# jihun1998/AO

Measured on AMD Instinct MI355X. Metric: points/sec fwd+bwd PTv2m2 S3DIS, higher is better.
Workload: dtype fp32

## Files before the change

ao_amd/csrc/abi.hip:

```cpp
#include <algorithm>
#include <cstdlib>
#include <cstring>
#include <mutex>
#include <unordered_map>
#include <vector>

#include "gva_common.h"

extern "C" int ptv2_abi_version(void) { return 11; }

extern "C" long long ptv2_struct_bytes(int which) {
    switch (which) {
        case 0: return (long long)sizeof(ptv2_block);
        case 1: return (long long)sizeof(ptv2_block_grads);
        case 2: return (long long)sizeof(ptv2_model);
        case 3: return (long long)sizeof(ptv2_gva_block);
        case 4: return (long long)sizeof(ptv2_scene_geo);
        default: return -1;
    }
}

namespace { thread_local int g_matmul_bf16 = 0; }
int ptv2_matmul_bf16(void) { return g_matmul_bf16; }
void ptv2_set_matmul_bf16(int on) { g_matmul_bf16 = on ? 1 : 0; }
// ... 74 lines not shown
        if (ids[r] < 0 || ids[r] >= dst_rows) return PTV2_ERR_ARG;
    for (long long r = 0; r < rows; ++r) memcpy(dst + ids[r] * c, src + r * c, sizeof(float) * (size_t)c);
    return PTV2_OK;
}

namespace {
std::mutex g_cnt_mu;
struct CounterKey {
    int device;
    hipStream_t stream;
    bool operator==(const CounterKey &o) const { return device == o.device && stream == o.stream; }
};
struct CounterKeyHash {
    size_t operator()(const CounterKey &k) const { return std::hash<void *>()((void *)k.stream) * 31u + (size_t)k.device; }
};
std::unordered_map<CounterKey, unsigned *, CounterKeyHash> g_counters;
}

unsigned *ptv2_stream_counters(hipStream_t st) {
    int device = 0;
    if (hipGetDevice(&device) != hipSuccess) return nullptr;
    std::lock_guard<std::mutex> lk(g_cnt_mu);
    const CounterKey key{device, st};
    auto it = g_counters.find(key);
    if (it != g_counters.end()) return it->second;
    unsigned *p = nullptr;
    if (hipMalloc((void **)&p, sizeof(unsigned) * PTV2_NUM_COUNTERS) != hipSuccess) return nullptr;
    if (hipMemsetAsync(p, 0, sizeof(unsigned) * PTV2_NUM_COUNTERS, st) != hipSuccess) return nullptr;
    g_counters[key] = p;
    return p;
}

namespace {
const char *kNames[KID_COUNT] = {
    "knn_row_query_kernel [family]", "logits_fwd_kernel [family]", "softmax_rows_kernel [family]", "aggregate_tile_kernel [family]",
    "peb_fwd_kernel [family]", "peb_bwd_kernel<8>", "aggregate_bwd_tile_kernel [family]", "aggregate_bwd_rows_kernel [family]",
    "aggregate_bwd_gv_kernel<8>", "logits_bwd_rows_kernel [family]", "logits_bwd_gather_kernel", "logits_bwd_params_kernel [family]",
    "linear_wgrad_kernel [family]", "bn_stats_kernel", "bn_apply_kernel [family]", "bn_bwd_reduce_kernel [family]",
    "bn_bwd_apply_kernel [family]", "skinny_fwd_kernel", "skinny_bwd_kernel", "rows_gemm_kernel<48, false, 32> [family]",
    "rows_gemm_kernel<48, false, 64> [family]", "rows_gemm_kernel<48, true, 32> [family]", "rows_gemm_kernel<48, true, 64> [family]",
    "rows_gemm_kernel<64, false, 32> [family]", "rows_gemm_kernel<64, false, 64> [family]", "rows_gemm_kernel<64, true, 32> [family]",
    "rows_gemm_kernel<64, true, 64> [family]",
    "attention_bwd_point_kernel<6, 48, 1, true>",
    "attention_bwd_point_kernel<12, 96, 1, false>", "attention_bwd_point_kernel<24, 192, 2, false>",
    "attention_bwd_point_kernel<48, 384, 4, false>", "attention_bwd_point_kernel<64, 512, 4, false>",
    "linear_wgrad_lds_kernel [family]",
    "grouped_wgrad_kernel_jobs", "attention_fwd_point6_kernel",
    "logits_bwd_fused6_kernel<48>", "logits_bwd_fused_kernel<12, 96, 1>", "logits_bwd_fused_kernel<24, 192, 4>",
    "logits_bwd_fused_kernel<48, 384, 4>", "logits_bwd_fused_kernel<64, 512, 4>",
    "bn_bwd_apply_residual_kernel", "bn_bwd_finapply_kernel [family]",
    "attention_fwd_tile_kernel<12, 96, 12>", "attention_fwd_tile_kernel<24, 192, 12>", "attention_fwd_tile_kernel<48, 384, 12>",
    "attention_fwd_tile_kernel<64, 512, 16>", "wp2_wgrad_tile_kernel_jobs",
    "attention_bwd_tile_kernel<12, 96, 8>", "attention_bwd_tile_kernel<24, 192, 8>", "attention_bwd_tile_kernel<48, 384, 8>",
    "attention_bwd_tile_kernel<64, 512, 8>"};
struct Rec { hipEvent_t a, b; double bytes; };
std::mutex g_mu;
int g_on = 0;
int g_only = -1;
int g_stride = 1;
unsigned g_seen[KID_COUNT];
std::vector<hipEvent_t> g_free;
hipEvent_t take_event() {
    if (!g_free.empty()) { hipEvent_t e = g_free.back(); g_free.pop_back(); return e; }
    hipEvent_t e = nullptr;
    if (hipEventCreate(&e) != hipSuccess) return nullptr;
    return e;
}
std::vector<Rec> g_recs[KID_COUNT];
std::vector<hipEvent_t> g_pending[KID_COUNT];
constexpr int STAMP_CAP = 1 << 15;
unsigned long long *g_stamp_buf = nullptr;
double g_stamp_us_per_tick = 0.01;
int g_stamp_n = 0;
struct StampRec { int slot; double bytes; };
std::vector<StampRec> g_stamp_recs[KID_COUNT];
std::vector<int> g_stamp_pending[KID_COUNT];
unsigned g_scope_period[GRAPH_SLOTS][KID_COUNT];
unsigned g_scope_phase[GRAPH_SLOTS];
thread_local unsigned t_scope_seen[KID_COUNT];
thread_local int t_scope_which = -1;
__global__ void stamp_kernel(unsigned long long *p) {
    if (threadIdx.x == 0) *p = wall_clock64();
}
}

extern "C" int ptv2_profile_is_on(void) { return g_on; }
int ptv2_profile_stamps(void) { return g_on && g_only >= 0 && g_stamp_buf != nullptr; }
void ptv2_profile_scope(int which, int end, int ring_entry, int ring_size) {
    if (which < 0 || which >= GRAPH_SLOTS) return;
    std::lock_guard<std::mutex> lk(g_mu);
    if (!end) {
        for (int k = 0; k < KID_COUNT; ++k) t_scope_seen[k] = 0;
        t_scope_which = which;
        const int stride = g_stride > 1 ? g_stride : 1;
        g_scope_phase[which] = (unsigned)(ring_entry * std::max(1, stride / std::max(1, ring_size)));
    } else {
        for (int k = 0; k < KID_COUNT; ++k) g_scope_period[which][k] = t_scope_seen[k];
        t_scope_which = -1;
    }
}
int ptv2_profile_wants(int kid) {
    if (!g_on || (g_only >= 0 && g_only != kid)) return 0;
    std::lock_guard<std::mutex> lk(g_mu);
    if (ptv2_graph_capturing() && t_scope_which >= 0) {
        const unsigned o = t_scope_seen[kid]++, P = g_scope_period[t_scope_which][kid], ph = g_scope_phase[t_scope_which];
        const unsigned stride = g_stride > 1 ? (unsigned)g_stride : 1u;
        return (P > 0 ? ((o + ph) % P) % stride : o % stride) == 0;
// ... 136 lines not shown
```

ao_amd/csrc/common.h:

```cpp
#pragma once
#include <hip/hip_runtime.h>
#include <stdint.h>
#include <stdlib.h>

#include "../../include/ptv2_hip.h"

#define WAVE 64

#define PTV2_CHECK_LAUNCH()                         \
    do {                                            \
        if (hipGetLastError() != hipSuccess) return PTV2_ERR_LAUNCH; \
    } while (0)

#define RUN(call)                        \
    do {                                 \
        int rc_ = (call);                \
        if (rc_ != PTV2_OK) return rc_;  \
    } while (0)

static inline int divup(long long a, long long b) { return (int)((a + b - 1) / b); }

static constexpr size_t ptv2_align256(size_t v) { return (v + 255) & ~(size_t)255; }
struct PtvCarver {
    char *p; size_t off;
    char *take(size_t bytes) { char *r = p ? p + off : nullptr; off += ptv2_align256(bytes); return r; }
    template <class T> T *take_n(size_t count) { return (T *)take(sizeof(T) * count); }
};

static inline bool ptv2_env_set(const char *name) { return getenv(name) != nullptr; }
static inline bool ptv2_env_is(const char *name, char c) { const char *e = getenv(name); return e && e[0] == c; }

enum PtvKernelId {
    KID_KNN_QUERY = 0, KID_LOGITS_FWD, KID_SOFTMAX_ROWS, KID_AGG_TILE, KID_PEB_FWD, KID_PEB_BWD, KID_BWD_TILE,
    KID_BWD_ROWS, KID_BWD_GV, KID_LOGITS_BWD_ROWS, KID_LOGITS_BWD_GATHER, KID_LOGITS_BWD_PARAMS, KID_WGRAD,
    KID_BN_STATS, KID_BN_APPLY, KID_BN_BWD_REDUCE, KID_BN_BWD_APPLY, KID_SKINNY_FWD, KID_SKINNY_BWD, KID_ROWS_GEMM,  KID_BWD_POINT = KID_ROWS_GEMM + 8,
     KID_WGRAD_LDS = KID_BWD_POINT + 5 ,
    KID_WGRAD_GROUPED ,
    KID_FWD_POINT ,
    KID_LOGITS_BWD_FUSED ,
    KID_BN_BWD_APPLY_RES = KID_LOGITS_BWD_FUSED + 5 ,
    KID_BN_BWD_FINAPPLY ,
    KID_FWD_TILE ,
    KID_WGRAD_TILE = KID_FWD_TILE + 4 ,
    KID_BWD_TILE_K ,
    KID_COUNT = KID_BWD_TILE_K + 4
};
extern "C" int ptv2_profile_is_on(void);
int ptv2_profile_wants(int kid);
void ptv2_profile_begin(int kid, hipStream_t st);
void ptv2_profile_end(int kid, hipStream_t st, double algorithmic_bytes);
struct PtvScopedTimer {
    int kid; hipStream_t st; double bytes; bool on;
    PtvScopedTimer(int k, hipStream_t s, double b) : kid(k), st(s), bytes(b), on(ptv2_profile_wants(k) != 0) {
        if (on) ptv2_profile_begin(kid, st);
    }
    ~PtvScopedTimer() { if (on) ptv2_profile_end(kid, st, bytes); }
};

enum PtvGraphSlot { GRAPH_MODEL_FWD = 0, GRAPH_MODEL_BWD = 1, GRAPH_MODEL_FWD_PREFIX = 2, GRAPH_MODEL_FWD_REST = 3, GRAPH_SLOTS = 4 };
struct PtvGraphScope {
    void *st, *cap; int which, ring_entry; bool active; long long t0;
    PtvGraphScope(void *stream, int which, bool allow = true);
    void *stream() const { return cap; }
    int finish(int rc);
    ~PtvGraphScope();
    PtvGraphScope(const PtvGraphScope &) = delete;
    PtvGraphScope &operator=(const PtvGraphScope &) = delete;
};
int ptv2_graph_capturing(void);
int ptv2_profile_stamps(void);
int ptv2_zero_async(void *p, size_t bytes, hipStream_t st);

void ptv2_wgrad_defer_begin(void *arena, size_t bytes);
bool ptv2_wgrad_defer_active();
float *ptv2_wgrad_defer_alloc(size_t floats);
void ptv2_wgrad_defer_arm(bool on);
void ptv2_wgrad_defer_arm_rs(bool on);
bool ptv2_wgrad_defer_armed_rs();
int ptv2_wgrad_defer_flush(void *stream);
void ptv2_wgrad_defer_end();
size_t ptv2_wgrad_defer_table_bytes();

int ptv2_matmul_bf16(void);
void ptv2_set_matmul_bf16(int on);
struct PtvMatmulScope {
    int prev;
    explicit PtvMatmulScope(int on) : prev(ptv2_matmul_bf16()) { ptv2_set_matmul_bf16(on); }
    ~PtvMatmulScope() { ptv2_set_matmul_bf16(prev); }
};
typedef __bf16 ptv2_bf16x8 __attribute__((ext_vector_type(8)));
__device__ __forceinline__ ptv2_bf16x8 ptv2_pack_bf16(float4 lo, float4 hi) {
    ptv2_bf16x8 r;
    r[0] = (__bf16)lo.x; r[1] = (__bf16)lo.y; r[2] = (__bf16)lo.z; r[3] = (__bf16)lo.w;
    r[4] = (__bf16)hi.x; r[5] = (__bf16)hi.y; r[6] = (__bf16)hi.z; r[7] = (__bf16)hi.w;
    return r;
}

static __device__ __attribute__((aligned(16), unused)) float ptv2_zero_pad[1024];
// ... 45 lines not shown
```

ao_amd/csrc/gemm.hip:

```cpp
#include <algorithm>

#include "common.h"

namespace gemm {

constexpr int BM = 64;
constexpr int THREADS = 256;
template <int KC>
__device__ __forceinline__ int lds_slot(int row, int k4) {
    return row * (KC + 8) + 4 * (k4 ^ (row & (KC == 32 ? 1 : 3)));
}

typedef float v4f __attribute__((ext_vector_type(4)));

struct GemmMulti {
    const float *X[3], *W[3], *bias[3];
    float *Y[3];
    int count;
    int sum;
    const float *xsc, *xsh;
    float *stats[3];
    const float *bnx, *bnm, *bnr, *bng, *bnb;
    int bnrelu;
    float *brec;
};

template <int CTRL>
__device__ __forceinline__ float dpp_mov(float v) {
    return __int_as_float(__builtin_amdgcn_update_dpp(0, __float_as_int(v), CTRL, 0xF, 0xF, true));
}
__device__ __forceinline__ float row16_sum(float v) {
    v += dpp_mov<0xB1>(v);
    v += dpp_mov<0x4E>(v);
    v += dpp_mov<0x141>(v);
    v += dpp_mov<0x140>(v);
    return v;
}

template <int BN>
__device__ __forceinline__ void gemm_epilogue(v4f (&acc)[BN / 16], const long long row0, const int rb, const int n0, const int z,
                                              const bool indep, const int m, const int n, const float *__restrict__ bias,
                                              float *__restrict__ Y, const int accumulate, const GemmMulti &multi, float *sS_) {
    constexpr int NT = BN / 16;
    const int tid = threadIdx.x, lane = tid & 63, wid = tid >> 6;
    float *sX = sS_;
    const long long row = row0 + wid * 16 + (lane & 15);
    float4 val[NT];
#pragma unroll
    for (int t = 0; t < NT; ++t) {
        const int col = n0 + t * 16 + (lane >> 4) * 4;
        float4 v = make_float4(acc[t][0], acc[t][1], acc[t][2], acc[t][3]);
        {
            const float4 bb = ptv2_ld_or_zero((const float4 *)(bias + col), bias && col < n);
            v.x += bb.x; v.y += bb.y; v.z += bb.z; v.w += bb.w;
        }
        val[t] = v;
        if (row < m && col < n) {
            float4 *dst = (float4 *)(Y + row * n + col);
            if (accumulate) {
                const float4 o = *dst;
                v.x += o.x; v.y += o.y; v.z += o.z; v.w += o.w;
            }
            *dst = v;
        }
    }
    if (multi.count && multi.brec) {
        float *sS = sX;
        const bool rv = row < m;
        const int cl = (lane >> 4) * 4;
        __syncthreads();
#pragma unroll
        for (int t = 0; t < NT; ++t) {
            const int col = n0 + t * 16 + cl;
            float4 d = make_float4(0.f, 0.f, 0.f, 0.f), e = d;
            if (rv && col < n) {
                const float4 xv = *(const float4 *)(multi.bnx + row * n + col);
                const float4 mm = *(const float4 *)(multi.bnm + col), rs = *(const float4 *)(multi.bnr + col);
                float4 h;
                h.x = (xv.x - mm.x) * rs.x; h.y = (xv.y - mm.y) * rs.y; h.z = (xv.z - mm.z) * rs.z; h.w = (xv.w - mm.w) * rs.w;
                d = val[t];
                if (multi.bnrelu) {
                    const float4 gg = *(const float4 *)(multi.bng + col), bb = *(const float4 *)(multi.bnb + col);
                    if (__builtin_fmaf(h.x, gg.x, bb.x) <= 0.f) d.x = 0.f;
                    if (__builtin_fmaf(h.y, gg.y, bb.y) <= 0.f) d.y = 0.f;
                    if (__builtin_fmaf(h.z, gg.z, bb.z) <= 0.f) d.z = 0.f;
                    if (__builtin_fmaf(h.w, gg.w, bb.w) <= 0.f) d.w = 0.f;
                }
                e = make_float4(d.x * h.x, d.y * h.y, d.z * h.z, d.w * h.w);
            }
            const float ax = row16_sum(d.x), ay = row16_sum(d.y), az = row16_sum(d.z), aw = row16_sum(d.w);
            const float bx = row16_sum(e.x), by = row16_sum(e.y), bz = row16_sum(e.z), bw = row16_sum(e.w);
            if ((lane & 15) == 0) {
                *(float4 *)(sS + (wid * 2 + 0) * BN + t * 16 + cl) = make_float4(ax, ay, az, aw);
                *(float4 *)(sS + (wid * 2 + 1) * BN + t * 16 + cl) = make_float4(bx, by, bz, bw);
            }
        }
        __syncthreads();
        for (int e = tid; e < 2 * BN; e += THREADS) {
            const int which = e / BN, cc = e - which * BN;
            if (n0 + cc < n) {
                float a = sS[which * BN + cc];
#pragma unroll
                for (int w = 1; w < 4; ++w) a += sS[(w * 2 + which) * BN + cc];
                multi.brec[(size_t)rb * 2 * n + (size_t)which * n + n0 + cc] = a;
            }
        }
// ... 1 lines not shown
    float *stats = multi.count ? multi.stats[indep ? z : 0] : nullptr;
    if (stats) {
        float *sS = sX;
        const bool rv = row < m;
        const int cnt = (int)((m - row0) < BM ? (m - row0) : BM);
        const int cl = (lane >> 4) * 4;
        __syncthreads();
#pragma unroll
        for (int t = 0; t < NT; ++t) {
            const float sx = row16_sum(rv ? val[t].x : 0.f), sy = row16_sum(rv ? val[t].y : 0.f);
            const float sz = row16_sum(rv ? val[t].z : 0.f), sw = row16_sum(rv ? val[t].w : 0.f);
            if ((lane & 15) == 0) *(float4 *)(sS + wid * BN + t * 16 + cl) = make_float4(sx, sy, sz, sw);
        }
        __syncthreads();
        float4 mean[NT];
#pragma unroll
        for (int t = 0; t < NT; ++t) {
            float4 a = *(const float4 *)(sS + t * 16 + cl);
#pragma unroll
            for (int w = 1; w < 4; ++w) {
                const float4 o = *(const float4 *)(sS + w * BN + t * 16 + cl);
                a.x += o.x; a.y += o.y; a.z += o.z; a.w += o.w;
            }
            mean[t] = a;
        }
        __syncthreads();
        const float inv = 1.0f / (float)cnt;
#pragma unroll
        for (int t = 0; t < NT; ++t) {
            const int col = n0 + t * 16 + cl;
            if (wid == 0 && (lane & 15) == 0 && col < n) *(float4 *)(stats + (size_t)rb * 2 * n + col) = mean[t];
            const float dx = rv ? val[t].x - mean[t].x * inv : 0.f, dy = rv ? val[t].y - mean[t].y * inv : 0.f;
            const float dz = rv ? val[t].z - mean[t].z * inv : 0.f, dw = rv ? val[t].w - mean[t].w * inv : 0.f;
            const float qx = row16_sum(dx * dx), qy = row16_sum(dy * dy), qz = row16_sum(dz * dz), qw = row16_sum(dw * dw);
            if ((lane & 15) == 0) *(float4 *)(sS + wid * BN + t * 16 + cl) = make_float4(qx, qy, qz, qw);
        }
        __syncthreads();
        if (wid == 0 && (lane & 15) == 0) {
#pragma unroll
            for (int t = 0; t < NT; ++t) {
                const int col = n0 + t * 16 + cl;
                if (col < n) {
                    float4 a = *(const float4 *)(sS + t * 16 + cl);
#pragma unroll
                    for (int w = 1; w < 4; ++w) {
                        const float4 o = *(const float4 *)(sS + w * BN + t * 16 + cl);
                        a.x += o.x; a.y += o.y; a.z += o.z; a.w += o.w;
                    }
                    *(float4 *)(stats + (size_t)rb * 2 * n + n + col) = a;
                }
            }
        }
    }
}

template <int BN, bool W_KMAJOR, int KC, bool BF16>
__global__ __launch_bounds__(THREADS) void rows_gemm_kernel(int m, int n, int k, const float *__restrict__ X0,
                                                            const float *__restrict__ W0,
                                                            const float *__restrict__ bias0, float *__restrict__ Y0,
                                                            int accumulate, int ncb, GemmMulti multi) {
    constexpr int PITCH = KC + 8;
    __shared__ __attribute__((aligned(16))) float sX[BM * PITCH];
    __shared__ __attribute__((aligned(16))) float sW[BN * PITCH];
    constexpr int NT = BN / 16;
    constexpr int KQ = KC / 4;
    constexpr int XLOADS = BM * KQ / THREADS;
    constexpr int WQ = BN * KQ;
    constexpr int WLOADS = (WQ + THREADS - 1) / THREADS;
    constexpr int RUN = KC / 16;
    const int tid = threadIdx.x, lane = tid & 63, wid = tid >> 6;
    const int rb = blockIdx.x / ncb, cb = blockIdx.x - rb * ncb;
    const long long row0 = (long long)rb * BM;
    const int n0 = cb * BN;
    const int z = blockIdx.y;
    const bool indep = multi.count && !multi.sum;
    const float *bias = indep ? multi.bias[z] : bias0;
    float *Y = multi.count ? multi.Y[indep ? z : 0] : Y0;
    const int npair = (multi.count && multi.sum) ? multi.count : 1;
    const float *X = multi.count ? multi.X[indep ? z : 0] : X0;
    const float *W = multi.count ? multi.W[indep ? z : 0] : W0;

    float4 rx[XLOADS], rw[WLOADS];
    auto fetch = [&](int k0) {
#pragma unroll
        for (int j = 0; j < XLOADS; ++j) {
            const int q = tid + j * THREADS, r = q / KQ, kq = (q % KQ) * 4;
            const long long row = row0 + r;
            rx[j] = ptv2_ld_or_zero((const float4 *)(X + row * k + k0 + kq), row < m && k0 + kq < k);
            if (multi.xsc && k0 + kq < k) {
                const float4 s4 = *(const float4 *)(multi.xsc + k0 + kq), h4 = *(const float4 *)(multi.xsh + k0 + kq);
                rx[j].x = fmaxf(__builtin_fmaf(rx[j].x, s4.x, h4.x), 0.f);
                rx[j].y = fmaxf(__builtin_fmaf(rx[j].y, s4.y, h4.y), 0.f);
                rx[j].z = fmaxf(__builtin_fmaf(rx[j].z, s4.z, h4.z), 0.f);
                rx[j].w = fmaxf(__builtin_fmaf(rx[j].w, s4.w, h4.w), 0.f);
            }
        }
#pragma unroll
        for (int j = 0; j < WLOADS; ++j) {
            const int q = tid + j * THREADS;
            {
                if (!W_KMAJOR) {
                    const int r = q / KQ, kq = (q % KQ) * 4;
                    rw[j] = ptv2_ld_or_zero((const float4 *)(W + (long long)(n0 + r) * k + k0 + kq), q < WQ && n0 + r < n && k0 + kq < k);
                } else {
                    const int kk = q % KC, cq = (q / KC) * 4;
                    rw[j] = ptv2_ld_or_zero((const float4 *)(W + (long long)(k0 + kk) * n + n0 + cq), q < WQ && k0 + kk < k && n0 + cq < n);
// ... 157 lines not shown
#pragma unroll
                for (int i = 0; i < 8; ++i) {
                    if (b0 + i < WL) {
                        const int e = tid + (b0 + i) * THREADS;
                        const int kk = e % K, cq = (e / K) * 4;
                        if (e < (BN / 4) * K) {
                            sW[(size_t)(cq + 0) * LDW + kk] = w4[i].x; sW[(size_t)(cq + 1) * LDW + kk] = w4[i].y;
                            sW[(size_t)(cq + 2) * LDW + kk] = w4[i].z; sW[(size_t)(cq + 3) * LDW + kk] = w4[i].w;
                        }
                    }
                }
            }
        }
        __syncthreads();
        if (multi.xsc) {
#pragma unroll
            for (int j = 0; j < QF; ++j) {
                const float4 s4 = *(const float4 *)(sSc + 16 * j + 4 * q), h4 = *(const float4 *)(sSc + K + 16 * j + 4 * q);
                x[j].x = fmaxf(__builtin_fmaf(x[j].x, s4.x, h4.x), 0.f); x[j].y = fmaxf(__builtin_fmaf(x[j].y, s4.y, h4.y), 0.f);
                x[j].z = fmaxf(__builtin_fmaf(x[j].z, s4.z, h4.z), 0.f); x[j].w = fmaxf(__builtin_fmaf(x[j].w, s4.w, h4.w), 0.f);
            }
        }
        const float *pw = sW + (size_t)l15 * LDW + 4 * q;
        if constexpr (BF16) {
#pragma unroll
            for (int j = 0; j < QF; j += 2) {
                const float4 x1 = j + 1 < QF ? x[j + 1] : make_float4(0.f, 0.f, 0.f, 0.f);
                const ptv2_bf16x8 xb = ptv2_pack_bf16(x[j], x1);
#pragma unroll
                for (int t = 0; t < NT; ++t) {
                    const float4 w0 = *(const float4 *)(pw + (size_t)t * 16 * LDW + 16 * j);
                    const float4 w1 = j + 1 < QF ? *(const float4 *)(pw + (size_t)t * 16 * LDW + 16 * (j + 1)) : make_float4(0.f, 0.f, 0.f, 0.f);
                    acc[t] = __builtin_amdgcn_mfma_f32_16x16x32_bf16(ptv2_pack_bf16(w0, w1), xb, acc[t], 0, 0, 0);
                }
            }
        } else {
#pragma unroll
            for (int j = 0; j < QF; ++j) {
#pragma unroll
                for (int t = 0; t < NT; ++t) {
                    const float4 w4 = *(const float4 *)(pw + (size_t)t * 16 * LDW + 16 * j);
                    acc[t] = __builtin_amdgcn_mfma_f32_16x16x4f32(w4.x, x[j].x, acc[t], 0, 0, 0);
                    acc[t] = __builtin_amdgcn_mfma_f32_16x16x4f32(w4.y, x[j].y, acc[t], 0, 0, 0);
                    acc[t] = __builtin_amdgcn_mfma_f32_16x16x4f32(w4.z, x[j].z, acc[t], 0, 0, 0);
                    acc[t] = __builtin_amdgcn_mfma_f32_16x16x4f32(w4.w, x[j].w, acc[t], 0, 0, 0);
                }
            }
        }
    }
    __syncthreads();
    gemm_epilogue<BN>(acc, row0, rb, n0, z, indep, m, n, bias, Y, accumulate, multi, sW);
}

template <int BN, bool W_KMAJOR, int K>
__global__ __launch_bounds__(THREADS) void rows_gemm_ksplit_kernel(int m, int n, const float *__restrict__ X0, const float *__restrict__ W0,
                                                                   const float *__restrict__ bias0, float *__restrict__ Y0, int accumulate,
                                                                   int ncb, GemmMulti multi) {
    constexpr int NT = BN / 16, QF = K / 16, JW = (QF + 3) / 4;
    __shared__ __attribute__((aligned(16))) float sRed[4][NT][64 * 4];
    const int tid = threadIdx.x, lane = tid & 63, wid = tid >> 6, l15 = lane & 15, q = lane >> 4;
    const int rb = blockIdx.x / ncb, cb = blockIdx.x - rb * ncb;
    const long long row0 = (long long)rb * 16;
    const int n0 = cb * BN;
    const int z = blockIdx.y;
    const bool indep = multi.count && !multi.sum;
    const float *bias = indep ? multi.bias[z] : bias0;
    float *Y = multi.count ? multi.Y[indep ? z : 0] : Y0;
    const int npair = (multi.count && multi.sum) ? multi.count : 1;
    const long long row = row0 + l15;
    const bool rv = row < m;
    const int j0 = wid * JW;
    v4f acc[NT];
#pragma unroll
    for (int t = 0; t < NT; ++t) acc[t] = (v4f){0.f, 0.f, 0.f, 0.f};
    for (int pair = 0; pair < npair; ++pair) {
        const float *X = multi.count ? multi.X[indep ? z : pair] : X0;
        const float *W = multi.count ? multi.W[indep ? z : pair] : W0;
        float4 x[JW], w[JW][NT], s4[JW], h4[JW];
        const float *xr = rv ? X + row * K + 4 * q : ptv2_zero_pad;
#pragma unroll
        for (int jj = 0; jj < JW; ++jj) {
            const int j = j0 + jj;
            const bool jok = j < QF;
            x[jj] = *(const float4 *)((jok && rv) ? xr + 16 * j : ptv2_zero_pad);
            if (multi.xsc) {
                s4[jj] = *(const float4 *)(jok ? multi.xsc + 16 * j + 4 * q : ptv2_zero_pad);
                h4[jj] = *(const float4 *)(jok ? multi.xsh + 16 * j + 4 * q : ptv2_zero_pad);
            }
#pragma unroll
            for (int t = 0; t < NT; ++t) {
                const int col = n0 + 16 * t + l15;
                const bool ok = jok && col < n;
                if (!W_KMAJOR) {
                    w[jj][t] = *(const float4 *)(ok ? W + (long long)col * K + 16 * j + 4 * q : ptv2_zero_pad);
                } else {
                    const float *wp = ok ? W + (long long)(16 * j + 4 * q) * n + col : ptv2_zero_pad;
                    const long long st = ok ? n : 0;
                    w[jj][t] = make_float4(wp[0], wp[st], wp[2 * st], wp[3 * st]);
                }
            }
        }
#pragma unroll
        for (int jj = 0; jj < JW; ++jj) {
            if (multi.xsc) {
                x[jj].x = fmaxf(__builtin_fmaf(x[jj].x, s4[jj].x, h4[jj].x), 0.f); x[jj].y = fmaxf(__builtin_fmaf(x[jj].y, s4[jj].y, h4[jj].y), 0.f);
                x[jj].z = fmaxf(__builtin_fmaf(x[jj].z, s4[jj].z, h4[jj].z), 0.f); x[jj].w = fmaxf(__builtin_fmaf(x[jj].w, s4[jj].w, h4[jj].w), 0.f);
// ... 56 lines not shown
            const float ax = row16_sum(d.x), ay = row16_sum(d.y), az = row16_sum(d.z), aw = row16_sum(d.w);
            const float bx = row16_sum(e.x), by = row16_sum(e.y), bz = row16_sum(e.z), bw = row16_sum(e.w);
            if (l15 == 0 && cok) {
                *(float4 *)(multi.brec + (size_t)rb * 2 * n + col) = make_float4(ax, ay, az, aw);
                *(float4 *)(multi.brec + (size_t)rb * 2 * n + n + col) = make_float4(bx, by, bz, bw);
            }
        }
        if (stats) {
            const float sx = row16_sum(rv ? val.x : 0.f), sy = row16_sum(rv ? val.y : 0.f);
            const float sz = row16_sum(rv ? val.z : 0.f), sw = row16_sum(rv ? val.w : 0.f);
            const float dx = rv ? val.x - sx * inv : 0.f, dy = rv ? val.y - sy * inv : 0.f;
            const float dz = rv ? val.z - sz * inv : 0.f, dw = rv ? val.w - sw * inv : 0.f;
            const float qx = row16_sum(dx * dx), qy = row16_sum(dy * dy), qz = row16_sum(dz * dz), qw = row16_sum(dw * dw);
            if (l15 == 0 && cok) {
                *(float4 *)(stats + (size_t)rb * 2 * n + col) = make_float4(sx, sy, sz, sw);
                *(float4 *)(stats + (size_t)rb * 2 * n + n + col) = make_float4(qx, qy, qz, qw);
            }
        }
    }
}

}

template <int BN, bool KM, int K>
static void launch_direct(dim3 grid, hipStream_t st, int m, int n, const float *X, const float *W, const float *bias, float *Y,
                          int accumulate, int ncb, const gemm::GemmMulti &gm) {
    const size_t lds = sizeof(float) * ((size_t)BN * (K + 8) + 2 * K);
    if (ptv2_matmul_bf16()) {
        auto kern = gemm::rows_gemm_direct_kernel<BN, KM, K, true>;
        if (lds > 48 * 1024) (void)hipFuncSetAttribute((const void *)kern, hipFuncAttributeMaxDynamicSharedMemorySize, (int)lds);
        hipLaunchKernelGGL(kern, grid, dim3(gemm::THREADS), lds, st, m, n, X, W, bias, Y, accumulate, ncb, gm);
    } else {
        auto kern = gemm::rows_gemm_direct_kernel<BN, KM, K, false>;
        if (lds > 48 * 1024) (void)hipFuncSetAttribute((const void *)kern, hipFuncAttributeMaxDynamicSharedMemorySize, (int)lds);
        hipLaunchKernelGGL(kern, grid, dim3(gemm::THREADS), lds, st, m, n, X, W, bias, Y, accumulate, ncb, gm);
    }
}

static bool launch_gemm_direct(int bn, bool kmajor, dim3 grid, hipStream_t st, int m, int n, int k, const float *X, const float *W,
                               const float *bias, float *Y, int accumulate, int ncb, const gemm::GemmMulti &gm) {
    const char *e = getenv("AO_AMD_GEMM");
    if ((e && e[0] == 'l') || (bn != 16 && bn != 48) || (k != 48 && k != 96 && k != 192 && k != 384)) return false;
    if (!(e && e[0] == 'd') && !(k == 48 || (!kmajor && bn == 48 && k <= 192))) return false;
#define GD(BN, KM, KK) launch_direct<BN, KM, KK>(grid, st, m, n, X, W, bias, Y, accumulate, ncb, gm)
#define GDK(BN, KM)                                                                   \
    switch (k) { case 48: GD(BN, KM, 48); break; case 96: GD(BN, KM, 96); break; case 192: GD(BN, KM, 192); break; default: GD(BN, KM, 384); break; }
    if (bn == 16) { if (kmajor) { GDK(16, true) } else { GDK(16, false) } }
    else { if (kmajor) { GDK(48, true) } else { GDK(48, false) } }
#undef GDK
#undef GD
    return true;
}

template <int BN, bool KM, int KC>
static void launch_one(dim3 grid, hipStream_t st, int m, int n, int k, const float *X, const float *W, const float *bias, float *Y,
                       int accumulate, int ncb, const gemm::GemmMulti &gm) {
    if (ptv2_matmul_bf16())
        hipLaunchKernelGGL((gemm::rows_gemm_kernel<BN, KM, KC, true>), grid, dim3(gemm::THREADS), 0, st, m, n, k, X, W, bias, Y,
                           accumulate, ncb, gm);
    else
        hipLaunchKernelGGL((gemm::rows_gemm_kernel<BN, KM, KC, false>), grid, dim3(gemm::THREADS), 0, st, m, n, k, X, W, bias, Y,
                           accumulate, ncb, gm);
}

static int column_block(int m, int n, int products = 1) {
    const bool n48 = n % 48 == 0;
    const int wide = n48 ? 48 : 64;
    const long long rbs = ((long long)m + gemm::BM - 1) / gemm::BM, prod = products;
    const long long wgs = rbs * ((n + wide - 1) / wide) * prod;
    constexpr int wide_min = 768;
    if (wgs >= wide_min || n % 16 != 0) return wide;
    constexpr int mid = 256;
    if (n % 32 == 0 && rbs * (n / 32) * prod >= mid) return 32;
    return 16;
}

namespace {
thread_local int g_rb16_ok = 0;
}
void ptv2_gemm_allow_rb16(int on) { g_rb16_ok = on; }
static bool ksplit_ok(int m, int n, int k, bool has_records) {
    static const bool on = ptv2_env_is("AO_AMD_GEMM_KSPLIT", '1');
    if (!on || ptv2_env_set("AO_AMD_GEMM") || ptv2_matmul_bf16()) return false;
    if (has_records && !g_rb16_ok) return false;
    return m >= 1 && m <= 32768 && (k == 96 || k == 192 || k == 384) && n % 16 == 0 && n >= 16;
}
int rows_gemm_record_rows(int m, int n, int k) { return ksplit_ok(m, n, k, true) ? 16 : 64; }

template <int BN, bool KM>
static void launch_ksplit_k(int k, dim3 grid, hipStream_t st, int m, int n, const float *X, const float *W, const float *bias, float *Y,
                            int accumulate, int ncb, const gemm::GemmMulti &gm) {
    switch (k) {
        case 96: hipLaunchKernelGGL((gemm::rows_gemm_ksplit_kernel<BN, KM, 96>), grid, dim3(gemm::THREADS), 0, st, m, n, X, W, bias, Y, accumulate, ncb, gm); break;
        case 192: hipLaunchKernelGGL((gemm::rows_gemm_ksplit_kernel<BN, KM, 192>), grid, dim3(gemm::THREADS), 0, st, m, n, X, W, bias, Y, accumulate, ncb, gm); break;
        default: hipLaunchKernelGGL((gemm::rows_gemm_ksplit_kernel<BN, KM, 384>), grid, dim3(gemm::THREADS), 0, st, m, n, X, W, bias, Y, accumulate, ncb, gm); break;
    }
}
static bool try_ksplit(int m, int n, int k, bool kmajor, int products, hipStream_t st, const float *X, const float *W, const float *bias,
                       float *Y, int accumulate, const gemm::GemmMulti &gm, bool has_records) {
    if (!ksplit_ok(m, n, k, has_records)) return false;
    const int bn = n % 48 == 0 ? 48 : (n % 64 == 0 ? 64 : (n % 32 == 0 ? 32 : 16));
    const int ncb = n / bn;
    const long long wgs = (((long long)m + 15) / 16) * ncb;
    if (wgs > 2147483647LL) return false;
    const dim3 grid((unsigned)wgs, (unsigned)products);
#define KS(BNN) do { if (kmajor) launch_ksplit_k<BNN, true>(k, grid, st, m, n, X, W, bias, Y, accumulate, ncb, gm); \
                     else launch_ksplit_k<BNN, false>(k, grid, st, m, n, X, W, bias, Y, accumulate, ncb, gm); } while (0)
    if (bn == 48) KS(48); else if (bn == 64) KS(64); else if (bn == 32) KS(32); else KS(16);
#undef KS
    return true;
}

static void launch_gemm(int bn, bool kmajor, bool wide_k, dim3 grid, hipStream_t st, int m, int n, int k, const float *X,
                        const float *W, const float *bias, float *Y, int accumulate, int ncb, const gemm::GemmMulti &gm) {
    if (launch_gemm_direct(bn, kmajor, grid, st, m, n, k, X, W, bias, Y, accumulate, ncb, gm)) return;
#define GO(BN, KM, KC) launch_one<BN, KM, KC>(grid, st, m, n, k, X, W, bias, Y, accumulate, ncb, gm)
    if (bn == 16) {
        if (kmajor) { if (wide_k) GO(16, true, 64); else GO(16, true, 32); }
        else { if (wide_k) GO(16, false, 64); else GO(16, false, 32); }
    } else if (bn == 32) {
        if (kmajor) { if (wide_k) GO(32, true, 64); else GO(32, true, 32); }
        else { if (wide_k) GO(32, false, 64); else GO(32, false, 32); }
    } else if (bn == 48) {
        if (kmajor) { if (wide_k) GO(48, true, 64); else GO(48, true, 32); }
        else { if (wide_k) GO(48, false, 64); else GO(48, false, 32); }
    } else {
        if (kmajor) { if (wide_k) GO(64, true, 64); else GO(64, true, 32); }
        else { if (wide_k) GO(64, false, 64); else GO(64, false, 32); }
    }
#undef GO
}

extern "C" int rows_gemm_hip_launcher(int m, int n, int k, const float *X, const float *W, int w_kmajor,
                                      const float *bias, float *Y, int accumulate, void *stream) {
    using namespace gemm;
    if (m < 0 || n < 4 || k < 4 || n % 4 != 0 || k % 4 != 0 || !X || !W || !Y) return PTV2_ERR_ARG;
    if (m == 0) return PTV2_OK;
    hipStream_t st = (hipStream_t)stream;
    const bool n48 = n % 48 == 0;
    const int bn = column_block(m, n);
    const int ncb = (n + bn - 1) / bn;
    const long long nrb = ((long long)m + BM - 1) / BM;
    if (nrb * ncb > 2147483647LL) return PTV2_ERR_ARG;
    const dim3 grid((unsigned)(nrb * ncb));
    {
        PtvScopedTimer t(KID_ROWS_GEMM + (n48 ? 0 : 4) + (w_kmajor ? 2 : 0) + (k >= 192 ? 1 : 0), st,
                         4.0 * ((double)m * (n + k) + (double)n * k));
        if (!try_ksplit(m, n, k, w_kmajor != 0, 1, st, X, W, bias, Y, accumulate, GemmMulti{}, false))
            launch_gemm(bn, w_kmajor != 0, k >= 192, grid, st, m, n, k, X, W, bias, Y, accumulate, ncb, GemmMulti{});
    }
    PTV2_CHECK_LAUNCH();
    return PTV2_OK;
}

extern "C" int rows_gemm_fused_hip_launcher(int m, int n, int k, int count, int sum, const float *const *X,
                                            const float *const *W, int w_kmajor, const float *const *bias, float *const *Y,
                                            int accumulate, const float *xsc, const float *xsh, float *const *stats,
                                            void *stream) {
    using namespace gemm;
    if (m < 0 || n < 4 || k < 4 || n % 4 != 0 || k % 4 != 0 || count < 1 || count > 3 || !X || !W || !Y) return PTV2_ERR_ARG;
    if (m == 0) return PTV2_OK;
    GemmMulti gm{};
    gm.count = count;
    gm.sum = sum ? 1 : 0;
    for (int i = 0; i < count; ++i) {
        if (!X[i] || !W[i] || (!Y[i] && (i == 0 || !sum))) return PTV2_ERR_ARG;
        gm.X[i] = X[i]; gm.W[i] = W[i]; gm.bias[i] = bias ? bias[i] : nullptr; gm.Y[i] = Y[i];
        gm.stats[i] = stats ? stats[i] : nullptr;
    }
    if ((xsc == nullptr) != (xsh == nullptr)) return PTV2_ERR_ARG;
    gm.xsc = xsc;
    gm.xsh = xsh;
    hipStream_t st = (hipStream_t)stream;
    const bool n48 = n % 48 == 0;
    const int bn = column_block(m, n, sum ? 1 : count);
    const int ncb = (n + bn - 1) / bn;
    const long long nrb = ((long long)m + BM - 1) / BM;
    if (nrb * ncb > 2147483647LL) return PTV2_ERR_ARG;
    const dim3 grid((unsigned)(nrb * ncb), sum ? 1 : count);
    const float *b0 = sum ? gm.bias[0] : nullptr;
    {
        PtvScopedTimer t(KID_ROWS_GEMM + (n48 ? 0 : 4) + (w_kmajor ? 2 : 0) + (k >= 192 ? 1 : 0), st,
                         4.0 * count * ((double)m * (n + k) + (double)n * k));
        bool records = false;
        for (int i = 0; i < count; ++i) records = records || gm.stats[i] != nullptr;
        if (!try_ksplit(m, n, k, w_kmajor != 0, sum ? 1 : count, st, gm.X[0], gm.W[0], b0, gm.Y[0], accumulate, gm, records))
            launch_gemm(bn, w_kmajor != 0, k >= 192, grid, st, m, n, k, gm.X[0], gm.W[0], b0, gm.Y[0], accumulate, ncb, gm);
    }
    PTV2_CHECK_LAUNCH();
    return PTV2_OK;
}

extern "C" int rows_gemm_multi_hip_launcher(int m, int n, int k, int count, int sum, const float *const *X,
                                            const float *const *W, int w_kmajor, const float *const *bias, float *const *Y,
                                            int accumulate, void *stream) {
    return rows_gemm_fused_hip_launcher(m, n, k, count, sum, X, W, w_kmajor, bias, Y, accumulate, nullptr, nullptr, nullptr,
                                        stream);
}

extern "C" int rows_gemm_bnbwd_hip_launcher(int m, int n, int k, int count, const float *const *X, const float *const *W,
                                            int w_kmajor, float *Y, const float *bn_x, const float *bn_mean, const float *bn_rstd,
                                            const float *bn_gamma, const float *bn_beta, int relu, float *records, void *stream) {
    using namespace gemm;
    if (m < 0 || n < 4 || k < 4 || n % 4 != 0 || k % 4 != 0 || count < 1 || count > 3 || !X || !W || !Y) return PTV2_ERR_ARG;
    if (!bn_x || !bn_mean || !bn_rstd || !records || (relu && (!bn_gamma || !bn_beta))) return PTV2_ERR_ARG;
    if (m == 0) return PTV2_OK;
    GemmMulti gm{};
    gm.count = count;
    gm.sum = 1;
    for (int i = 0; i < count; ++i) {
        if (!X[i] || !W[i]) return PTV2_ERR_ARG;
        gm.X[i] = X[i]; gm.W[i] = W[i];
    }
    gm.Y[0] = Y;
    gm.bnx = bn_x; gm.bnm = bn_mean; gm.bnr = bn_rstd; gm.bng = bn_gamma; gm.bnb = bn_beta; gm.bnrelu = relu; gm.brec = records;
    hipStream_t st = (hipStream_t)stream;
    const bool n48 = n % 48 == 0;
    const int bn = column_block(m, n);
    const int ncb = (n + bn - 1) / bn;
    const long long nrb = ((long long)m + BM - 1) / BM;
    if (nrb * ncb > 2147483647LL) return PTV2_ERR_ARG;
    const dim3 grid((unsigned)(nrb * ncb), 1);
    {
        PtvScopedTimer t(KID_ROWS_GEMM + (n48 ? 0 : 4) + (w_kmajor ? 2 : 0) + (k >= 192 ? 1 : 0), st,
                         4.0 * ((double)m * (2 * n + count * k) + (double)count * n * k));
        if (!try_ksplit(m, n, k, w_kmajor != 0, 1, st, gm.X[0], gm.W[0], nullptr, Y, 0, gm, true))
            launch_gemm(bn, w_kmajor != 0, k >= 192, grid, st, m, n, k, gm.X[0], gm.W[0], nullptr, Y, 0, ncb, gm);
    }
    PTV2_CHECK_LAUNCH();
    return PTV2_OK;
}
```

Before: 12.88 million.

## Add persistent rows GEMM kernel for 48x48 products with LDS-resident weights

Adds a persistent-grid GEMM kernel for n=k=48 that stages the weight matrices into LDS once per workgroup. Each workgroup then loops over row blocks, prefetching the next block's X rows into registers while computing the current one, and reuses a shared epilogue that now takes preloaded bias. It is enabled only when there are more row blocks than resident workgroups and operands are not summed pairs. The aim is to avoid reloading W for every row block and to cut launch and tail overhead. In exchange it adds register pressure, an occupancy query, and a wider dispatch surface including the bnbwd path.

```diff
diff --git a/ao_amd/csrc/abi.hip b/ao_amd/csrc/abi.hip
--- a/ao_amd/csrc/abi.hip
+++ b/ao_amd/csrc/abi.hip
@@ -150,7 +150,7 @@
     "attention_fwd_tile_kernel<12, 96, 12>", "attention_fwd_tile_kernel<24, 192, 12>", "attention_fwd_tile_kernel<48, 384, 12>",
     "attention_fwd_tile_kernel<64, 512, 16>", "wp2_wgrad_tile_kernel_jobs",
     "attention_bwd_tile_kernel<12, 96, 8>", "attention_bwd_tile_kernel<24, 192, 8>", "attention_bwd_tile_kernel<48, 384, 8>",
-    "attention_bwd_tile_kernel<64, 512, 8>"};
+    "attention_bwd_tile_kernel<64, 512, 8>", "rows_gemm_persist_kernel [family]"};
 struct Rec { hipEvent_t a, b; double bytes; };
 std::mutex g_mu;
 int g_on = 0;
diff --git a/ao_amd/csrc/common.h b/ao_amd/csrc/common.h
--- a/ao_amd/csrc/common.h
+++ b/ao_amd/csrc/common.h
@@ -43,7 +43,8 @@
     KID_FWD_TILE ,
     KID_WGRAD_TILE = KID_FWD_TILE + 4 ,
     KID_BWD_TILE_K ,
-    KID_COUNT = KID_BWD_TILE_K + 4
+    KID_ROWS_GEMM_PERSIST = KID_BWD_TILE_K + 4 ,
+    KID_COUNT
 };
 extern "C" int ptv2_profile_is_on(void);
 int ptv2_profile_wants(int kid);
diff --git a/ao_amd/csrc/gemm.hip b/ao_amd/csrc/gemm.hip
--- a/ao_amd/csrc/gemm.hip
+++ b/ao_amd/csrc/gemm.hip
@@ -38,9 +38,9 @@
 }
 
 template <int BN>
-__device__ __forceinline__ void gemm_epilogue(v4f (&acc)[BN / 16], const long long row0, const int rb, const int n0, const int z,
-                                              const bool indep, const int m, const int n, const float *__restrict__ bias,
-                                              float *__restrict__ Y, const int accumulate, const GemmMulti &multi, float *sS_) {
+__device__ __forceinline__ void gemm_epilogue_bb(v4f (&acc)[BN / 16], const long long row0, const int rb, const int n0, const int z,
+                                                 const bool indep, const int m, const int n, const float4 (&bb_)[BN / 16],
+                                                 float *__restrict__ Y, const int accumulate, const GemmMulti &multi, float *sS_) {
     constexpr int NT = BN / 16;
     const int tid = threadIdx.x, lane = tid & 63, wid = tid >> 6;
     float *sX = sS_;
@@ -51,7 +51,7 @@
         const int col = n0 + t * 16 + (lane >> 4) * 4;
         float4 v = make_float4(acc[t][0], acc[t][1], acc[t][2], acc[t][3]);
         {
-            const float4 bb = ptv2_ld_or_zero((const float4 *)(bias + col), bias && col < n);
+            const float4 bb = bb_[t];
             v.x += bb.x; v.y += bb.y; v.z += bb.z; v.w += bb.w;
         }
         val[t] = v;
@@ -159,6 +159,19 @@
             }
         }
     }
+}
+
+template <int BN>
+__device__ __forceinline__ void gemm_epilogue(v4f (&acc)[BN / 16], const long long row0, const int rb, const int n0, const int z,
+                                              const bool indep, const int m, const int n, const float *__restrict__ bias,
+                                              float *__restrict__ Y, const int accumulate, const GemmMulti &multi, float *sS_) {
+    float4 bb[BN / 16];
+#pragma unroll
+    for (int t = 0; t < BN / 16; ++t) {
+        const int col = n0 + t * 16 + ((threadIdx.x & 63) >> 4) * 4;
+        bb[t] = ptv2_ld_or_zero((const float4 *)(bias + col), bias && col < n);
+    }
+    gemm_epilogue_bb<BN>(acc, row0, rb, n0, z, indep, m, n, bb, Y, accumulate, multi, sS_);
 }
 
 template <int BN, bool W_KMAJOR, int KC, bool BF16>
@@ -422,6 +435,122 @@
     gemm_epilogue<BN>(acc, row0, rb, n0, z, indep, m, n, bias, Y, accumulate, multi, sW);
 }
 
+template <bool W_KMAJOR>
+__device__ __forceinline__ void persist_stage_w(float *sW, const float *__restrict__ W) {
+    constexpr int K = 48, BN = 48, LDW = K + 8, KQ = K / 4, Q = BN * KQ, WL = (Q + THREADS - 1) / THREADS;
+    const int tid = threadIdx.x;
+    float4 w4[WL];
+#pragma unroll
+    for (int i = 0; i < WL; ++i) {
+        const int e = tid + i * THREADS;
+        if (!W_KMAJOR) {
+            w4[i] = ptv2_ld_or_zero((const float4 *)(W + 4 * e), e < Q);
+        } else {
+            const int kk = e % K, cq = (e / K) * 4;
+            w4[i] = ptv2_ld_or_zero((const float4 *)(W + kk * BN + cq), e < Q);
+        }
+    }
+#pragma unroll
+    for (int i = 0; i < WL; ++i) {
+        const int e = tid + i * THREADS;
+        if (e < Q) {
+            if (!W_KMAJOR) {
+                const int r = e / KQ, k4 = e - r * KQ;
+                *(float4 *)(sW + r * LDW + 4 * k4) = w4[i];
+            } else {
+                const int kk = e % K, cq = (e / K) * 4;
+                sW[(cq + 0) * LDW + kk] = w4[i].x; sW[(cq + 1) * LDW + kk] = w4[i].y;
+                sW[(cq + 2) * LDW + kk] = w4[i].z; sW[(cq + 3) * LDW + kk] = w4[i].w;
+            }
+        }
+    }
+}
+
+template <bool W_KMAJOR, int NPAIR, int NPROD>
+__global__ __launch_bounds__(THREADS) void rows_gemm_persist_kernel(int m, int nrb, const float *__restrict__ X0,
+                                                                    const float *__restrict__ W0, const float *__restrict__ bias0,
+                                                                    float *__restrict__ Y0, int accumulate, GemmMulti multi) {
+    static_assert(NPAIR == 1 || NPROD == 1, "summed pairs or independent products");
+    constexpr int K = 48, BN = 48, NT = BN / 16, QF = K / 16, LDW = K + 8, NW = NPAIR * NPROD;
+    extern __shared__ float4 gp_lds4[];
+    float *sW = (float *)gp_lds4;
+    float *sSc = sW + NW * BN * LDW;
+    float *sE = sSc + 2 * K;
+    float *sB = sE + 4 * 2 * BN;
+    const int tid = threadIdx.x, lane = tid & 63, wid = tid >> 6, l15 = lane & 15, q = lane >> 4;
+    const bool indep = multi.count && !multi.sum;
+
+#pragma unroll
+    for (int w = 0; w < NW; ++w) persist_stage_w<W_KMAJOR>(sW + w * BN * LDW, multi.count ? multi.W[w] : W0);
+    if (multi.xsc)
+        for (int e = tid; e < K; e += THREADS) { sSc[e] = multi.xsc[e]; sSc[K + e] = multi.xsh[e]; }
+    for (int e = tid; e < NPROD * BN; e += THREADS) {
+        const float *bias = indep ? multi.bias[e / BN] : bias0;
+        sB[e] = bias ? bias[e % BN] : 0.f;
+    }
+
+    auto request = [&](float4 (&x)[NPAIR][QF], long long rb) {
+        const long long row = rb * BM + wid * 16 + l15;
+#pragma unroll
+        for (int p = 0; p < NPAIR; ++p) {
+            const float *X = multi.count ? multi.X[p] : X0;
+            const float *xr = row < m ? X + row * K + 4 * q : ptv2_zero_pad;
+#pragma unroll
+            for (int j = 0; j < QF; ++j) x[p][j] = *(const float4 *)(xr + 16 * j);
+        }
+    };
+    float4 xn[NPAIR][QF];
+    request(xn, blockIdx.x);
+    __syncthreads();
+    const float *pw = sW + l15 * LDW + 4 * q;
+    for (int rb = blockIdx.x; rb < nrb; rb += gridDim.x) {
+        float4 x[NPAIR][QF];
+#pragma unroll
+        for (int p = 0; p < NPAIR; ++p)
+#pragma unroll
+            for (int j = 0; j < QF; ++j) x[p][j] = xn[p][j];
+        request(xn, (long long)rb + gridDim.x);
+        if (multi.xsc) {
+#pragma unroll
+            for (int j = 0; j < QF; ++j) {
+                const float4 s4 = *(const float4 *)(sSc + 16 * j + 4 * q), h4 = *(const float4 *)(sSc + K + 16 * j + 4 * q);
+#pragma unroll
+                for (int p = 0; p < NPAIR; ++p) {
+                    float4 &v = x[p][j];
+                    v.x = fmaxf(__builtin_fmaf(v.x, s4.x, h4.x), 0.f); v.y = fmaxf(__builtin_fmaf(v.y, s4.y, h4.y), 0.f);
+                    v.z = fmaxf(__builtin_fmaf(v.z, s4.z, h4.z), 0.f); v.w = fmaxf(__builtin_fmaf(v.w, s4.w, h4.w), 0.f);
+                }
+            }
+        }
+#pragma unroll
+        for (int z = 0; z < NPROD; ++z) {
+            v4f acc[NT];
+#pragma unroll
+            for (int t = 0; t < NT; ++t) acc[t] = (v4f){0.f, 0.f, 0.f, 0.f};
+#pragma unroll
+            for (int p = 0; p < NPAIR; ++p) {
+                const float *pwz = pw + (NPROD > 1 ? z : p) * BN * LDW;
+#pragma unroll
+                for (int j = 0; j < QF; ++j) {
+#pragma unroll
+                    for (int t = 0; t < NT; ++t) {
+                        const float4 w4 = *(const float4 *)(pwz + t * 16 * LDW + 16 * j);
+                        acc[t] = __builtin_amdgcn_mfma_f32_16x16x4f32(w4.x, x[p][j].x, acc[t], 0, 0, 0);
+                        acc[t] = __builtin_amdgcn_mfma_f32_16x16x4f32(w4.y, x[p][j].y, acc[t], 0, 0, 0);
+                        acc[t] = __builtin_amdgcn_mfma_f32_16x16x4f32(w4.z, x[p][j].z, acc[t], 0, 0, 0);
+                        acc[t] = __builtin_amdgcn_mfma_f32_16x16x4f32(w4.w, x[p][j].w, acc[t], 0, 0, 0);
+                    }
+                }
+            }
+            float4 bb[NT];
+#pragma unroll
+            for (int t = 0; t < NT; ++t) bb[t] = *(const float4 *)(sB + z * BN + t * 16 + 4 * q);
+            float *Y = multi.count ? multi.Y[indep ? z : 0] : Y0;
+            gemm_epilogue_bb<BN>(acc, (long long)rb * BM, rb, 0, z, indep, m, BN, bb, Y, accumulate, multi, sE);
+        }
+    }
+}
+
 template <int BN, bool W_KMAJOR, int K>
 __global__ __launch_bounds__(THREADS) void rows_gemm_ksplit_kernel(int m, int n, const float *__restrict__ X0, const float *__restrict__ W0,
                                                                    const float *__restrict__ bias0, float *__restrict__ Y0, int accumulate,
@@ -584,6 +713,70 @@
     return true;
 }
 
+template <bool KM, int NPAIR, int NPROD>
+static int persist_resident() {
+    static const int resident = [] {
+        int dev = 0, cus = 0, per_cu = 0;
+        const size_t lds = sizeof(float) * ((size_t)NPAIR * NPROD * 48 * 56 + 2 * 48 + 4 * 2 * 48 + NPROD * 48);
+        if (hipGetDevice(&dev) != hipSuccess || hipDeviceGetAttribute(&cus, hipDeviceAttributeMultiprocessorCount, dev) != hipSuccess ||
+            hipOccupancyMaxActiveBlocksPerMultiprocessor(&per_cu, (const void *)gemm::rows_gemm_persist_kernel<KM, NPAIR, NPROD>,
+                                                         gemm::THREADS, lds) != hipSuccess) {
+            (void)hipGetLastError();
+            return 0;
+        }
+        return cus * per_cu;
+    }();
+    return resident;
+}
+template <bool KM, int NPAIR, int NPROD>
+static void launch_persist_one(int grid, hipStream_t st, int m, int nrb, const float *X, const float *W, const float *bias, float *Y,
+                               int accumulate, const gemm::GemmMulti &gm) {
+    const size_t lds = sizeof(float) * ((size_t)NPAIR * NPROD * 48 * 56 + 2 * 48 + 4 * 2 * 48 + NPROD * 48);
+    hipLaunchKernelGGL((gemm::rows_gemm_persist_kernel<KM, NPAIR, NPROD>), dim3((unsigned)grid), dim3(gemm::THREADS), lds, st, m, nrb, X, W,
+                       bias, Y, accumulate, gm);
+}
+static int persist_dispatch(bool kmajor, int npair, int nprod, int grid, hipStream_t st, int m, int nrb, const float *X, const float *W,
+                            const float *bias, float *Y, int accumulate, const gemm::GemmMulti &gm) {
+#define PS(KM, NPAIR, NPROD)                                                                          \
+    do {                                                                                              \
+        if (grid <= 0) return persist_resident<KM, NPAIR, NPROD>();                                   \
+        launch_persist_one<KM, NPAIR, NPROD>(grid, st, m, nrb, X, W, bias, Y, accumulate, gm);        \
+        return grid;                                                                                  \
+    } while (0)
+#define PSK(KM)                                                                   \
+    do {                                                                          \
+        if (npair == 3) PS(KM, 3, 1); else if (npair == 2) PS(KM, 2, 1);          \
+        else if (nprod == 3) PS(KM, 1, 3); else if (nprod == 2) PS(KM, 1, 2);     \
+        else PS(KM, 1, 1);                                                        \
+    } while (0)
+    if (kmajor) PSK(true); else PSK(false);
+    return 0;
+#undef PSK
+#undef PS
+}
+static bool persist_pays(long long nrb, int resident, int npair, int nprod) {
+    (void)nprod;
+    return npair == 1 && nrb > resident;
+}
+static int persist_grid(int m, int n, int k, bool kmajor, const gemm::GemmMulti &gm, int *npair, int *nprod) {
+    if (n != 48 || k != 48 || ptv2_matmul_bf16() || ptv2_env_set("AO_AMD_GEMM") || ptv2_env_is("AO_AMD_GEMM_PERSIST", '0'))
+        return 0;
+    *npair = (gm.count && gm.sum) ? gm.count : 1;
+    *nprod = (gm.count && !gm.sum) ? gm.count : 1;
+    for (int i = 1; i < *nprod; ++i)
+        if (gm.X[i] != gm.X[0]) return 0;
+    const long long nrb = ((long long)m + gemm::BM - 1) / gemm::BM;
+    const int resident = persist_dispatch(kmajor, *npair, *nprod, 0, nullptr, 0, 0, nullptr, nullptr, nullptr, nullptr, 0, gm);
+    if (resident <= 0) return 0;
+    const char *cap_s = getenv("AO_AMD_GEMM_PERSIST_WGS");
+    const long long cap = cap_s ? atoll(cap_s) : 0;
+    const bool forced = cap > 0 || ptv2_env_is("AO_AMD_GEMM_PERSIST", '1');
+    if (!forced && !persist_pays(nrb, resident, *npair, *nprod)) return 0;
+    if (cap > 0) return (int)std::min(nrb, cap);
+    const long long trips = (nrb + resident - 1) / resident;
+    return (int)((nrb + trips - 1) / trips);
+}
+
 template <int BN, bool KM, int KC>
 static void launch_one(dim3 grid, hipStream_t st, int m, int n, int k, const float *X, const float *W, const float *bias, float *Y,
                        int accumulate, int ncb, const gemm::GemmMulti &gm) {
@@ -676,9 +869,13 @@
     if (nrb * ncb > 2147483647LL) return PTV2_ERR_ARG;
     const dim3 grid((unsigned)(nrb * ncb));
     {
-        PtvScopedTimer t(KID_ROWS_GEMM + (n48 ? 0 : 4) + (w_kmajor ? 2 : 0) + (k >= 192 ? 1 : 0), st,
+        int npair = 1, nprod = 1;
+        const int pg = persist_grid(m, n, k, w_kmajor != 0, GemmMulti{}, &npair, &nprod);
+        PtvScopedTimer t(pg ? KID_ROWS_GEMM_PERSIST : KID_ROWS_GEMM + (n48 ? 0 : 4) + (w_kmajor ? 2 : 0) + (k >= 192 ? 1 : 0), st,
                          4.0 * ((double)m * (n + k) + (double)n * k));
-        if (!try_ksplit(m, n, k, w_kmajor != 0, 1, st, X, W, bias, Y, accumulate, GemmMulti{}, false))
+        if (pg)
+            persist_dispatch(w_kmajor != 0, 1, 1, pg, st, m, (int)nrb, X, W, bias, Y, accumulate, GemmMulti{});
+        else if (!try_ksplit(m, n, k, w_kmajor != 0, 1, st, X, W, bias, Y, accumulate, GemmMulti{}, false))
             launch_gemm(bn, w_kmajor != 0, k >= 192, grid, st, m, n, k, X, W, bias, Y, accumulate, ncb, GemmMulti{});
     }
     PTV2_CHECK_LAUNCH();
@@ -712,11 +909,16 @@
     const dim3 grid((unsigned)(nrb * ncb), sum ? 1 : count);
     const float *b0 = sum ? gm.bias[0] : nullptr;
     {
-        PtvScopedTimer t(KID_ROWS_GEMM + (n48 ? 0 : 4) + (w_kmajor ? 2 : 0) + (k >= 192 ? 1 : 0), st,
-                         4.0 * count * ((double)m * (n + k) + (double)n * k));
+        int npair = 1, nprod = 1;
+        const int pg = persist_grid(m, n, k, w_kmajor != 0, gm, &npair, &nprod);
+        PtvScopedTimer t(pg ? KID_ROWS_GEMM_PERSIST : KID_ROWS_GEMM + (n48 ? 0 : 4) + (w_kmajor ? 2 : 0) + (k >= 192 ? 1 : 0), st,
+                         pg && nprod > 1 ? 4.0 * ((double)m * (count * n + k) + (double)count * n * k)
+                                         : 4.0 * count * ((double)m * (n + k) + (double)n * k));
         bool records = false;
         for (int i = 0; i < count; ++i) records = records || gm.stats[i] != nullptr;
-        if (!try_ksplit(m, n, k, w_kmajor != 0, sum ? 1 : count, st, gm.X[0], gm.W[0], b0, gm.Y[0], accumulate, gm, records))
+        if (pg)
+            persist_dispatch(w_kmajor != 0, npair, nprod, pg, st, m, (int)nrb, gm.X[0], gm.W[0], b0, gm.Y[0], accumulate, gm);
+        else if (!try_ksplit(m, n, k, w_kmajor != 0, sum ? 1 : count, st, gm.X[0], gm.W[0], b0, gm.Y[0], accumulate, gm, records))
             launch_gemm(bn, w_kmajor != 0, k >= 192, grid, st, m, n, k, gm.X[0], gm.W[0], b0, gm.Y[0], accumulate, ncb, gm);
     }
     PTV2_CHECK_LAUNCH();
@@ -754,9 +956,13 @@
     if (nrb * ncb > 2147483647LL) return PTV2_ERR_ARG;
     const dim3 grid((unsigned)(nrb * ncb), 1);
     {
-        PtvScopedTimer t(KID_ROWS_GEMM + (n48 ? 0 : 4) + (w_kmajor ? 2 : 0) + (k >= 192 ? 1 : 0), st,
+        int npair = 1, nprod = 1;
+        const int pg = persist_grid(m, n, k, w_kmajor != 0, gm, &npair, &nprod);
+        PtvScopedTimer t(pg ? KID_ROWS_GEMM_PERSIST : KID_ROWS_GEMM + (n48 ? 0 : 4) + (w_kmajor ? 2 : 0) + (k >= 192 ? 1 : 0), st,
                          4.0 * ((double)m * (2 * n + count * k) + (double)count * n * k));
-        if (!try_ksplit(m, n, k, w_kmajor != 0, 1, st, gm.X[0], gm.W[0], nullptr, Y, 0, gm, true))
+        if (pg)
+            persist_dispatch(w_kmajor != 0, npair, nprod, pg, st, m, (int)nrb, gm.X[0], gm.W[0], nullptr, Y, 0, gm);
+        else if (!try_ksplit(m, n, k, w_kmajor != 0, 1, st, gm.X[0], gm.W[0], nullptr, Y, 0, gm, true))
             launch_gemm(bn, w_kmajor != 0, k >= 192, grid, st, m, n, k, gm.X[0], gm.W[0], nullptr, Y, 0, ncb, gm);
     }
     PTV2_CHECK_LAUNCH();
```

Measured after the change: 12.86 million. No clear change (-0.1%).
